# arpg/ba

Hardware: AMD Instinct MI355X
Metric: Gauss-Newton iterations/sec (higher is better)
Workload: dtype f64; 1 GPU; BASELINE.json configs[3]: 10000 poses / 1000000 landmarks / 10000000 reprojection residuals, pinhole, LmSize=1, PoseSize=6, Gauss-Newton (no dogleg), 2 anchor poses inactive; poses=10000, landmarks=1000000, residuals=10000000, reduced_system_n=59988, driver=phase calls of the C-ABI (include/ba_hip.h), parallelism=single GPU

## Files before the change

### ba_amd/csrc/engine.h

```cpp
#pragma once
#include <hip/hip_runtime.h>
#include <stdint.h>
#include <string>
#include <vector>

#include "../../include/ba_hip.h"
#include "structure.h"
#include "ordering.h"
#include "selinv.h"
#include "marg.h"
#include "pcg.h"
#include "dist_plan.h"

namespace bae {

template <typename T>
struct DBuf {
  T* p = nullptr;
  size_t n = 0;
  hipError_t alloc(size_t count) {
    if (count <= n && p) return hipSuccess;
    release();
    if (count == 0) { n = 0; return hipSuccess; }
    hipError_t err = hipMalloc((void**)&p, count * sizeof(T));
    if (err == hipSuccess) n = count;
    return err;
  }
  void release() {
    if (p) (void)hipFree(p);
    p = nullptr;
    n = 0;
  }
  size_t bytes() const { return n * sizeof(T); }
};
template <typename T>
// ... 69 lines not shown
  DBuf<double> obs_w0;
  DBuf<uint8_t> obs_cond;
  DBuf<uint2> wave_rng;
  DBuf<uint32_t> tile_ptr;
  DBuf<uint2> tile_ref;
  DBuf<uint32_t> tile_order;
  DBuf<uint4> tile_desc;
  uint32_t n_tile_order = 0;
  uint64_t tile_order_version = ~0ull;
  uint64_t tile_order_plan = ~0ull;
  int dbg_assemble_variant = 5;
  int dbg_host_structure = 0;
  int dbg_linearize_variant = 0;
  int dbg_tile_order = 0;
  int dbg_imu_wave = -1;
  int dbg_all_tiles = 0;
  DBuf<uint2> pair_ent;
  DBuf<uint32_t> pose_ptr, pose_mid;
  DBuf<uint32_t> pose_ent;
  DBuf<uint8_t> nzL;
  bool nzL_valid = false;
  std::vector<uint8_t> nzL_host;
  uint64_t nzL_version = 0;
  std::vector<uint8_t> nzS_host;
  DBuf<uint32_t> dist_srows;
  std::vector<uint32_t> dist_srows_off;
  uint64_t dist_srows_version = ~0ull;
  DBuf<uint32_t> dist_rows;
  std::vector<uint32_t> dist_rows_off;
  uint64_t dist_rows_version = ~0ull;
  DBuf<double> dist_msg;
  DistPlan dist_plan;
  uint64_t dist_plan_version = ~0ull;
  std::string dist_layout_name;
  DBuf<uint32_t> dist_tiles;
  uint64_t dist_sp_version = ~0ull;
  std::vector<uint32_t> dist_sp_send, dist_sp_recv;
  std::vector<size_t> dist_sp_send_off, dist_sp_recv_off;
  DBuf<uint4> dist_sp_srect, dist_sp_rrect;
  DBuf<uint2> dist_pairs;
  std::vector<uint32_t> dist_pair_first;
  uint32_t dist_npairs = 0;
  DBuf<uint32_t> dist_sq_list;
  DBuf<double> dist_usend, dist_urecv;
  DBuf<double> dist_ssend, dist_srecv;
  DBuf<double> dist_back;
// ... 203 lines not shown
int launch_calib_border(Engine* e);
int launch_calib_dogleg(Engine* e, int gn_available, ba_hip_dogleg_scalars* out);
int launch_begin_solve(Engine* e);
int launch_end_solve(Engine* e);
int launch_residual_vectors(Engine* e, double* d_r2);
int launch_residuals(Engine* e, int mode);
int launch_landmarks(Engine* e, double c_huber, int use_robust);
int launch_gather_S(Engine* e);
int launch_pack_lower(Engine* e, int unpack);
size_t packed_lower_count(uint32_t n_pad);
int launch_backsub(Engine* e);
int launch_compose_step(Engine* e, double coef_rhs, double coef_gn, double* norms2_host);
int launch_apply_step(Engine* e);
int launch_dogleg(Engine* e, int gn_available, double* h7, bool skip_jrhs);
int select_kth(Engine* e, const double* d_values, uint32_t n_local, uint64_t k, double* out);
int sum_partials(Engine* e, uint32_t nparts, uint32_t ncomp, double* host_out, bool cross_shard = true);
void defer_begin(Engine* e);
int defer_flush(Engine* e);
int launch_imu_early(Engine* e, double c_huber_proj);
int launch_posepose_build(Engine* e, double c_huber_proj, double* h3);
int launch_posepose_eval(Engine* e, double* h3);
int launch_posepose_jrhs(Engine* e, double* out);
int cholesky_solve(Engine* e, double* dA, uint32_t n, uint32_t ld, double* dx, int* status,
                   const uint8_t* nz_tiles);
int factor_tile_pattern(Engine* e);
uint32_t choose_kout(uint32_t nblk);
bool dist_solve_enabled(const Engine* e);
int dist_reduce_scatter_S(Engine* e);
int launch_imu_residual_vectors(Engine* e, double* d_r15);
int build_tile_order(Engine* e);
int build_tile_desc(Engine* e);
int dist_assembly_tiles(Engine* e, std::vector<uint8_t>* need);
int build_lists_device(Engine* e, const std::function<void(const char*)>& stage);
int order_poses(Engine* e, std::vector<uint64_t>* proj_edges, double device_ms);
bool ordering_wants_graph(const Engine* e);
int dist_broadcast(Engine* e, double* buf, size_t count, int root, hipStream_t s);
struct DistXfer { double* buf; size_t count; int peer; bool send; };
int dist_exchange(Engine* e, const std::vector<DistXfer>& x, bool side, hipStream_t s);
int dist_allreduce_stream(Engine* e, double* buf, size_t count, hipStream_t s);
void comm_release(Engine* e);
int check_solve_residual(Engine* e, const double* dS, const double* dx, const double* db, double* out2);
int cholesky_solve_dist(Engine* e, double* dA, uint32_t ld, double* dx, int* status, const uint8_t* nz);
int trailing_marginals(Engine* e, const double* dA, uint32_t ld, uint32_t first, uint32_t K, double* cov);
int marginals_compute(Engine* e);
int marginals_gather(Engine* e, uint32_t n, const std::vector<uint32_t>& ra, const std::vector<uint32_t>& rb, int Da,
                     int Db, double* out);
int marginals_landmarks(Engine* e, uint32_t n, const uint32_t* ids, double* out);
void marginals_release(Engine* e);
int leverages_run(Engine* e, uint32_t n, const uint32_t* ids, double* out);
// ... 14 lines not shown
```

### ba_amd/csrc/engine.hip

```cpp
#include "engine.h"
#include <chrono>
#include <functional>
#include <memory>
#include <thread>

#include <algorithm>
#include <cmath>
#include <cstdlib>
#include <cstring>
#include <numeric>

#include "dmath.h"
#include "dpose.h"

namespace bae {

int Engine::fail(hipError_t e, const char* what) {
  err = std::string(what) + ": " + hipGetErrorString(e);
  return -(int)(e == hipSuccess ? 1 : e);
}
void Engine::prof_collect() {
  auto drain = [](std::vector<std::pair<hipEvent_t, hipEvent_t>>& v, double& ms, uint32_t& n) {
    for (auto& p : v) {
      (void)hipEventSynchronize(p.second);
// ... 1020 lines not shown
      uint32_t a = 0;
      for (uint32_t p = 0; p < st.P; ++p)
        if (st.pose_opt[p] >= 0) {
          for (uint32_t d = 0; d < D; ++d) nat[(size_t)st.pose_opt[p] * D + d] = a * D + d;
          ++a;
        }
      for (uint32_t k = 0; k < st.K; ++k) nat[st.np + k] = st.Pact * D + k;
      build_pcg_coarse(e->pcg_plan, nat, st.Pact, D, st.K, e->pcg_opt.coarse_aggregate);
      e->pcg_coarse_built = e->pcg_opt.coarse_aggregate;
    }
    if ((rc = pcg_solve_device(e, e->A.p, st.n, st.ld, e->rhs_sc.p, e->pcg_plan, e->nzS_host, e->pcg_blk, e->pcg_blocks, rebuild,
                               e->pcg_opt, e->gn_p.p, &e->pcg_stats, &status))) return rc;
    e->factored = false;
    e->pcg_last = e->pcg_solved = true;
  } else if (st.n > 0 && !skip) {
    if (e->opt.keep_reduced_system) {
      BAE_HIP(e->A_keep.alloc((size_t)st.ld * st.ld));
      BAE_HIP(hipMemcpyAsync(e->A_keep.p, e->A.p, (size_t)st.ld * st.ld * sizeof(double),
                             hipMemcpyDeviceToDevice, e->stream));
    }
    if (!e->nzL_valid && (rc = factor_tile_pattern(e))) return rc;
    if (dist_solve_enabled(e)) {
      if ((rc = cholesky_solve_dist(e, e->A.p, st.ld, e->gn_p.p, &status, e->nzL.p))) return rc;
    } else if ((rc = cholesky_solve(e, e->A.p, st.n, st.ld, e->gn_p.p, &status, e->nzL.p))) return rc;
    e->factored = true;
    e->factor_foreign = false;
  }
  e->timers.solve = t.stop_ms();
  EventTimer tb(e);
  if ((rc = launch_backsub(e))) return rc;
  e->timers.back_substitution = tb.stop_ms();
  return status ? BA_HIP_FACTORIZATION_ERROR : 0;
}

int ba_hip_dogleg_terms(ba_hip_engine* h, int gn_available, ba_hip_dogleg_scalars* out) {
  ENG(h);
  NEED_FINAL();
  BAE_HIP(hipSetDevice(e->device));
  memset(out, 0, sizeof(*out));
  double* dh = e->dog_h;
  const bool reuse = gn_available && e->dog_jrhs_valid;
  defer_begin(e);
  int rc = launch_dogleg(e, gn_available, dh, reuse);
  if (!rc && !reuse) rc = launch_posepose_jrhs(e, dh + 7);
  if (!rc && !reuse) rc = launch_priors_jrhs(e, &e->prior_jrhs_h);
  const int rf = defer_flush(e);
  if (rc || rf) { e->dog_jrhs_valid = false; return rc ? rc : rf; }
// ... 669 lines not shown
  if (err != hipSuccess) rc = e->fail(err, "hipMemcpy");
  if (!rc && shard_allreduce(e, d.p, count, dtype) != 0) rc = e->fail_msg("allreduce hook failed");
  if (!rc && (err = hipMemcpy(host, d.p, count * 8, hipMemcpyDeviceToHost)) != hipSuccess) rc = e->fail(err, "hipMemcpy");
  d.release();
  return rc;
}

int ba_hip_get_comm_stats(ba_hip_engine* h, ba_hip_comm_stats* out) {
  ENG(h);
  if (!out) return e->fail_msg("null output");
  *out = e->cstats;
  return 0;
}

int ba_hip_reset_comm_stats(ba_hip_engine* h) {
  ENG(h);
  memset(&e->cstats, 0, sizeof(e->cstats));
  return 0;
}

int ba_hip_dist_plan_stats(uint32_t nblk, const uint8_t* nz_lower, int nranks, const char* layout, uint32_t kout,
                           ba_hip_dist_plan_stats_t* out) {
  if (!out || nranks < 1 || nblk == 0) return -1;
  const uint32_t G = kout ? kout : choose_kout(nblk);
  OwnMap map;
  std::string name;
  if (!build_own_map((uint32_t)nranks, layout, G, &map, &name)) return -1;
  const DistPlanStats s = dist_plan_stats(build_dist_plan(nblk, map, nz_lower));
  out->factor_bytes = s.factor_bytes;
  out->chain_recv_max = s.chain_recv_max; out->chain_recv_total = s.chain_recv_total;
  out->side_recv_max = s.side_recv_max; out->side_recv_total = s.side_recv_total;
  out->chain_sent_total = s.chain_sent_total; out->side_sent_total = s.side_sent_total;
  out->recv_max = s.recv_max; out->backward_allreduce_bytes = s.backward_allreduce_bytes;
  out->messages_chain = s.messages_chain; out->messages_side = s.messages_side;
  out->panels = s.panels; out->ranks = s.ranks; out->classes = s.classes; out->kout = G;
  return 0;
}

int ba_hip_get_factor_tile_pattern(ba_hip_engine* h, uint32_t nblk, uint8_t* nz_lower) {
  ENG(h);
  NEED_FINAL();
  if (!e->nzL_valid) {
    BAE_HIP(hipSetDevice(e->device));
    const int rc = factor_tile_pattern(e);
    if (rc) return rc;
  }
  if (e->nzL_host.size() != (size_t)nblk * nblk) return e->fail_msg("tile count mismatch");
  memcpy(nz_lower, e->nzL_host.data(), e->nzL_host.size());
  return 0;
}

int ba_hip_solve_is_distributed(ba_hip_engine* h) {
  if (!h) return 0;
  return dist_solve_enabled(reinterpret_cast<Engine*>(h)) ? 1 : 0;
}

int ba_hip_set_pose_ordering(ba_hip_engine* h, int mode) {
  ENG(h);
  if (mode != kOrderNatural && mode != kOrderAuto && mode != kOrderUser)
    return e->fail_msg("ba_hip_set_pose_ordering: unknown mode");
  if (mode != kOrderNatural && e->ordering_refused())
    return e->fail_msg("pose ordering is not available on a sharded engine (all-reduce hook, collectives hook or communicator set)");
  e->order_mode = mode;
  return 0;
}

int ba_hip_set_reduced_solver(ba_hip_engine* h, int mode, const ba_hip_pcg_options* o) {
  ENG(h);
  if (mode != BA_HIP_SOLVER_DIRECT && mode != BA_HIP_SOLVER_PCG) return e->fail_msg("ba_hip_set_reduced_solver: unknown mode");
  if (mode == BA_HIP_SOLVER_PCG) {
    if (e->pcg_refused())
      return e->fail_msg("the PCG solver is not available on a sharded engine (all-reduce hook, collectives hook or communicator set)");
    ba_hip_pcg_options v = {};
    v.rel_tolerance = 1e-6;
    if (o) v = *o;
    if (!(v.rel_tolerance > 0.0) || !(v.rel_tolerance < 1.0))
      return e->fail_msg("ba_hip_set_reduced_solver: rel_tolerance must lie in (0, 1)");
// ... 297 lines not shown
        if (!t && tile_map && r / 64 != c / 64) {
          e->err = "ba_hip_tile_solve: entry (" + std::to_string(r) + ", " + std::to_string(c) + ") is nonzero but tile (" +
                   std::to_string(r / 64) + ", " + std::to_string(c / 64) + ") is not in the tile map";
          return -1;
        }
        t = 1;
      }
    }
  for (uint32_t i = 0; i < nt; ++i) nz[(size_t)i * nt + i] = 1;
  for (uint32_t r = n; r < ld; ++r) A[(size_t)r * ld + r] = 1.0;
  for (uint32_t c = 0; c < n; ++c) A[(size_t)ld * ld + c] = b[c];
  tile_symbolic_factor(nz, nt);
  if (nz_factor) std::copy(nz.begin(), nz.end(), nz_factor);
  DBuf<double> dA, dx;
  DBuf<uint8_t> dnz;
  BAE_HIP(dA.alloc(A.size()));
  BAE_HIP(dx.alloc(ld));
  BAE_HIP(dnz.alloc(nz.size()));
  BAE_HIP(e->flags.alloc(16));
  BAE_HIP(hipMemcpy(dA.p, A.data(), A.size() * 8, hipMemcpyHostToDevice));
  BAE_HIP(hipMemcpy(dnz.p, nz.data(), nz.size(), hipMemcpyHostToDevice));
  int status = 0;
  e->factor_foreign = true;
  int rc = cholesky_solve(e, dA.p, n, ld, dx.p, &status, dnz.p);
  if (rc == 0) {
    std::vector<double> xx(ld);
    hipError_t err = hipDeviceSynchronize();
    if (err == hipSuccess) err = hipMemcpy(xx.data(), dx.p, (size_t)ld * 8, hipMemcpyDeviceToHost);
    if (err == hipSuccess && factor) err = hipMemcpy(factor, dA.p, (size_t)ld * ld * 8, hipMemcpyDeviceToHost);
    if (err == hipSuccess && dsgn) err = hipMemcpy(dsgn, e->invdiag.p, (size_t)ld * 8, hipMemcpyDeviceToHost);
    if (err == hipSuccess && linvT)
      err = hipMemcpy(linvT, e->invdiag.p + ld, (size_t)nt * 64 * 64 * 8, hipMemcpyDeviceToHost);
    if (err != hipSuccess) rc = e->fail(err, "hipMemcpy");
    for (uint32_t i = 0; i < n; ++i) x[i] = xx[i];
  }
  dA.release(); dx.release(); dnz.release();
  if (rc) return rc;
  return status ? BA_HIP_FACTORIZATION_ERROR : 0;
}

int ba_hip_select_kth(ba_hip_engine* h, uint32_t n, const double* values, uint32_t k, double* out) {
  ENG(h);
  BAE_HIP(hipSetDevice(e->device));
  DBuf<double> dv;
  BAE_HIP(dv.alloc(std::max<uint32_t>(n, 1)));
  BAE_HIP(e->hist.alloc(2048 + 8));
  if (n) BAE_HIP(hipMemcpy(dv.p, values, (size_t)n * 8, hipMemcpyHostToDevice));
// ... 7 lines not shown
```

### ba_amd/csrc/hostcheck.cpp

```cpp
#include <vector>
#include "dmath.h"
using namespace bad;

static Rt rt_from7(const double* p) {
  Rt t;
  t.R = quat_to_rot(p[3], p[4], p[5], p[6]);
  t.t = v3(p[0], p[1], p[2]);
  return t;
}

static double g_hostcheck_fov_w = 0.0;
extern "C" void ba_hostcheck_set_fov(double w) { g_hostcheck_fov_w = w; }
static Cam cam_from4(const double* cam4) {
  Cam c = {cam4[0], cam4[1], cam4[2], cam4[3], g_hostcheck_fov_w, g_hostcheck_fov_w != 0.0 ? 1 : 0};
  return c;
}

static int g_hostcheck_variant = 1;
extern "C" void ba_hostcheck_set_variant(int v) { g_hostcheck_variant = v; }

extern "C" void ba_hostcheck_proj_jacobians(int lm_dim, const double* cam4, const double* z,
                                            const double* x, const double* t_wp_m7,
                                            const double* t_vs_m7, const double* t_wp_r7,
                                            const double* t_vs_r7, int same_pose, double* r2,
// ... 575 lines not shown
        for (int x = 0; x < 6; ++x)
          rows[(WO + k) * 6 + x] = (rows[x] * Jl[k] + rows[6 + x] * Jl[LM + k]) * sw;
      if (LM == 1) {
        double* lr = &frow[((size_t)st.lrow_base + 2 * l) * 6];
        for (int x = 0; x < 6; ++x) lr[x] += (rows[12 + x] * Jl[0] + rows[18 + x] * Jl[1]) * sw;
      }
      if (K > 0)
        for (int x = 0; x < K; ++x)
          crow[(2 * (size_t)O + l) * 6 + x] += (crow[2 * (size_t)s * 6 + x] * Jl[0] + crow[(2 * (size_t)s + 1) * 6 + x] * Jl[1]) * sw;
    }
  }
  LeverHostIn in;
  in.LM = LM; in.D = D; in.K = K; in.L = L; in.O = O; in.np = st.np; in.n = st.n; in.lrow_base = st.lrow_base;
  in.lm_ptr = st.lm_ptr.data(); in.obs_pose = st.obs_pose.data(); in.lm_ref_pose = lm_ref_pose;
  in.pose_opt = st.pose_opt.data(); in.lm_opt = st.lm_opt.data();
  in.frow = frow.data(); in.obs_jl = obs_jl.data(); in.crow = K > 0 ? crow.data() : nullptr;
  in.sigma = sigma;
  std::vector<double> sorted((size_t)O * 4, 0.0);
  leverage_host(in, variant, sorted.data());
  for (uint32_t s = 0; s < O; ++s)
    for (int i = 0; i < 4; ++i) out[4 * (size_t)st.obs_perm[s] + i] = sorted[4 * (size_t)s + i];
  return 0;
}
```

### ba_amd/csrc/k_chol.hip

```cpp
#include "engine.h"
#include <cstdlib>
#include <algorithm>
#include <vector>

namespace bae {

static const int NB = 64;
static const int LDT = NB + 2;

typedef double double4_t __attribute__((ext_vector_type(4)));

__device__ __forceinline__ double readlane_f64(double v, int lane) {
  int lo = __double2loint(v), hi = __double2hiint(v);
  lo = __builtin_amdgcn_readlane(lo, lane);
  hi = __builtin_amdgcn_readlane(hi, lane);
  return __hiloint2double(hi, lo);
}

static const int LDM = 18;

static const int KC2 = 16;
#ifndef BAE_LDK2
#define BAE_LDK2 (KC2 + 2)
#endif
// ... 252 lines not shown
    while ((uint64_t)(sr + 1) * (sr + 2) / 2 <= t) ++sr;
    while ((uint64_t)sr * (sr + 1) / 2 > t) --sr;
    const uint32_t sc = t - (uint32_t)((uint64_t)sr * (sr + 1) / 2);
    const uint32_t R = (sr << sbl) + (within >> sbl), C = (sc << sbl) + (within & ((1u << sbl) - 1u));
    if (C > R) return;
    c = c0 + C;
    i = c0 + R;
    if (i > nblk || c >= nblk) return;
  } else {
    c = c0 + blockIdx.y;
    i = c + blockIdx.x;
    if (i > nblk) return;
  }
  if (!own_tile(own, i, c, nblk)) return;
  update_tile(A, ld, nblk, i, c, kb0, kb1, dsgn, colneg, nz, X, Y, klist);
}

static const int NB2 = 128;
#ifdef BAE_TIME128
__device__ unsigned long long* g_t128_buf = nullptr;
__device__ unsigned int g_t128_n = 0;
static const unsigned int T128_CAP = 1u << 21, T128_REC = 6;
#endif
template <bool RECT, bool LIST = false>
__global__ void __launch_bounds__(256, 2)
k_update128(double* __restrict__ A, uint32_t ld, uint32_t nblk, uint32_t c0, uint32_t m2, uint32_t kb0,
            uint32_t kb1, const double* __restrict__ dsgn, const int* __restrict__ colneg, uint32_t sbl,
            const uint8_t* __restrict__ nz, const OwnMap own,
            uint32_t nrow64, uint32_t r0, uint32_t rect_cols) {
  __shared__ double X[2][NB2][LDK2];
  __shared__ double Y[2][NB2][LDK2];
  __shared__ uint32_t klist[32];
  if (blockIdx.x < nrow64) {
    const uint32_t mcols = RECT ? 2 * rect_cols : nblk - c0, y = blockIdx.x / mcols;
    const uint32_t c = c0 + blockIdx.x % mcols, i = nblk - y;
    if (y > ((nblk - r0) & 1u) || c > i || c >= nblk) return;
    if (!own_tile(own, i, c, nblk)) return;
    update_tile(A, ld, nblk, i, c, kb0, kb1, dsgn, colneg, nz, reinterpret_cast<double(*)[NB][LDK2]>(&X[0][0][0]),
                reinterpret_cast<double(*)[NB][LDK2]>(&Y[0][0][0]), klist);
    return;
  }
  const uint32_t b = blockIdx.x - nrow64;
  uint32_t R, C;
  if constexpr (LIST) {
    const uint32_t gb = own.G >> 1, per = gb * gb;
    const uint32_t pr = b / per, within = b - pr * per;
    const uint2* pairs = reinterpret_cast<const uint2*>(((unsigned long long)own.pairs_hi << 32) | own.pairs_lo);
    const uint2 bp = pairs[pr];
    const uint32_t base = c0 / own.G;
    R = (bp.x - base) * gb + within / gb;
    C = (bp.y - base) * gb + within % gb;
    if (C > R || R >= m2) return;
  } else if (RECT) {
    R = b / rect_cols;
    C = b % rect_cols;
    if (R >= m2) return;
  } else {
    const uint32_t xcd = b & 7u, slot = b >> 3;
    const uint32_t t = (slot >> (2 * sbl)) * 8u + xcd, within = slot & ((1u << (2 * sbl)) - 1u);
    uint32_t sr_ = (uint32_t)((sqrt(8.0 * (double)t + 1.0) - 1.0) * 0.5);
    while ((uint64_t)(sr_ + 1) * (sr_ + 2) / 2 <= t) ++sr_;
    while ((uint64_t)sr_ * (sr_ + 1) / 2 > t) --sr_;
    const uint32_t sc_ = t - (uint32_t)((uint64_t)sr_ * (sr_ + 1) / 2);
    R = (sr_ << sbl) + (within >> sbl);
    C = (sc_ << sbl) + (within & ((1u << sbl) - 1u));
    if (C > R || R >= m2) return;
  }
// ... 964 lines not shown
  if (nz.size() != (size_t)nt * nt) nz.assign((size_t)nt * nt, 1);
  static const bool dense = getenv("BA_HIP_DENSE") != nullptr;
  if (dense) std::fill(nz.begin(), nz.end(), 1);
  if (e->sharded() && !dense) {
    std::vector<double> cnt(nz.begin(), nz.end());
    DBuf<double> d;
    BAE_HIP(d.alloc(cnt.size()));
    BAE_HIP(hipMemcpy(d.p, cnt.data(), cnt.size() * sizeof(double), hipMemcpyHostToDevice));
    if (shard_allreduce(e, d.p, cnt.size(), 0) != 0) { d.release(); return e->fail_msg("allreduce hook failed"); }
    BAE_HIP(hipMemcpy(cnt.data(), d.p, cnt.size() * sizeof(double), hipMemcpyDeviceToHost));
    d.release();
    for (size_t i = 0; i < nz.size(); ++i) nz[i] = cnt[i] > 0.5 ? 1 : 0;
  }
  e->nzS_host = nz;
  tile_symbolic_factor(nz, nt);
  BAE_HIP(e->nzL.alloc(nz.size()));
  BAE_HIP(hipMemcpy(e->nzL.p, nz.data(), nz.size(), hipMemcpyHostToDevice));
  e->nzL_host = nz;
  e->nzL_version++;
  e->nzL_valid = true;
  return 0;
}

uint32_t choose_kout(uint32_t nblk) {
  const char* ke = getenv("BA_HIP_KOUT");
  const uint32_t kout_env = ke ? (uint32_t)atoi(ke) : 0;
  return kout_env ? kout_env : (nblk >= 400 ? 16u : nblk >= 256 ? 8u : 4u);
}

bool dist_solve_enabled(const Engine* e) {
  static const bool off = getenv("BA_HIP_NO_DIST_SOLVE") != nullptr;
  return e->coll && e->sharded() && !e->opt.keep_reduced_system && !off;
}

__global__ void __launch_bounds__(256)
k_copy_panel_rows(double* __restrict__ A, uint32_t ld, const uint32_t* __restrict__ tiles, uint32_t ntiles,
                  uint32_t n_pad, uint32_t c0, uint32_t w, double* __restrict__ buf, int unpack) {
  const uint32_t r = blockIdx.x;
  const uint32_t arow = (r < ntiles * NB) ? tiles[r >> 6] * NB + (r & 63u) : n_pad;
  double* row = A + (size_t)arow * ld + c0;
  double* brow = buf + (size_t)r * w;
  for (uint32_t cc = threadIdx.x; cc < w; cc += 256) {
    if (unpack) row[cc] = brow[cc];
    else brow[cc] = row[cc];
  }
}

static const uint32_t KIN = 4;
static void launch_panel_chain(hipStream_t s, double* dA, uint32_t ld, uint32_t nblk, uint32_t J, uint32_t Jend,
                               double* dsgn, double* opbuf, int* colneg, int* flags, const uint8_t* nz,
// ... 54 lines not shown
                                     uint32_t ncols, uint32_t kb0, uint32_t kb1, double* dsgn, double* opbuf,
                                     int* colneg, int* flags, const uint8_t* nz, bool factor = true) {
  static const bool no128 = getenv("BA_HIP_NO128") != nullptr;
  const uint32_t r0 = c0 + ncols;
  auto step_update = factor ? k_step_update<true> : k_step_update<false>;
  static const uint32_t min_rows =
      getenv("BA_HIP_BULK_FULL_M") ? (uint32_t)std::max(16, atoi(getenv("BA_HIP_BULK_FULL_M"))) : 128u;
  if (!no128 && r0 + min_rows <= nblk && ncols % 2u == 0 && c0 % 2u == 0) {
    const uint32_t m = nblk - r0, m2 = m / 2, rect_cols = ncols / 2;
    hipLaunchKernelGGL(step_update, dim3(ncols, ncols), dim3(256), 0, s, dA, ld, nblk, c0, kb0, kb1, dsgn, opbuf,
                       colneg, flags, nz, r0, (const uint32_t*)nullptr);
    const uint32_t nrow64 = (ncols * (1 + (m & 1u)) + 7) / 8 * 8;
    hipLaunchKernelGGL(k_update128<true>, dim3(nrow64 + m2 * rect_cols), dim3(256), 0, s, dA, ld, nblk, c0, m2, kb0, kb1,
                       (const double*)dsgn, (const int*)colneg, 0u, nz, own_map_single(), nrow64, r0, rect_cols);
    return;
  }
  hipLaunchKernelGGL(step_update, dim3(nblk - c0 + 1, ncols), dim3(256), 0, s, dA, ld, nblk, c0, kb0, kb1, dsgn,
                     opbuf, colneg, flags, nz, nblk + 1u, (const uint32_t*)nullptr);
}

static void launch_bulk_update(Engine* e, hipStream_t s, double* dA, uint32_t ld, uint32_t nblk, uint32_t a_end,
                                   uint32_t J, uint32_t Jend, const double* dsgn, const int* colneg,
                                   const uint8_t* nz, bool full, const OwnMap& own, const uint2* pairs = nullptr,
                                   uint32_t npairs = 0) {
  static const bool no128 = getenv("BA_HIP_NO128") != nullptr;
  static const uint32_t sbl = getenv("BA_HIP_SBL") ? (uint32_t)atoi(getenv("BA_HIP_SBL")) : 3u;
  const uint32_t m = nblk - a_end;
  if (full && !no128 && m >= 16 && (a_end % 2u) == 0 && (own.n <= 1 || own.G % 2u == 0)) {
    const uint32_t m2 = m / 2, sbl2 = 2, sbe2 = 1u << sbl2;
    const uint32_t nsr = (m2 + sbe2 - 1) / sbe2, nsb = nsr * (nsr + 1) / 2;
    const uint32_t nrow64 = (m * (1 + (m & 1u)) + 7) / 8 * 8;
    if (e) e->prof_begin(e->ev_syrk, s);
    if (pairs && own.n > 1 && a_end % own.G == 0) {
      OwnMap ol = own;
      ol.pairs_lo = (uint32_t)(reinterpret_cast<unsigned long long>(pairs) & 0xffffffffull);
      ol.pairs_hi = (uint32_t)(reinterpret_cast<unsigned long long>(pairs) >> 32);
      const uint32_t per = (own.G / 2) * (own.G / 2);
      hipLaunchKernelGGL((k_update128<false, true>), dim3(nrow64 + npairs * per), dim3(256), 0, s, dA, ld, nblk,
                         a_end, m2, J, Jend, dsgn, colneg, sbl2, nz, ol, nrow64, a_end, 0u);
    } else {
      hipLaunchKernelGGL(k_update128<false>, dim3(nrow64 + ((nsb + 7) / 8) * 8 * sbe2 * sbe2), dim3(256), 0, s, dA, ld, nblk,
                         a_end, m2, J, Jend, dsgn, colneg, sbl2, nz, own, nrow64, a_end, 0u);
    }
    if (e) e->prof_end(e->ev_syrk, s);
    return;
  }
  const uint32_t sbe = 1u << sbl;
  const uint32_t nsr = (m + 1 + sbe - 1) / sbe, nsb = nsr * (nsr + 1) / 2;
  const uint32_t grid1 = ((nsb + 7) / 8) * 8 * sbe * sbe;
  const int swzf = 1 | (int)(sbl << 8);
  if (e) e->prof_begin(e->ev_syrk, s);
  if (full)
    hipLaunchKernelGGL(k_update2<false>, dim3(grid1), dim3(256), 0, s, dA, ld, nblk, a_end, J, Jend, dsgn, colneg,
                       swzf, nz, own);
  else
    hipLaunchKernelGGL(k_update2<true>, dim3(grid1), dim3(256), 0, s, dA, ld, nblk, a_end, J, Jend, dsgn, colneg,
                       swzf, nz, own);
  if (e) e->prof_end(e->ev_syrk, s);
}

static int ensure_dist_plan(Engine* e, uint32_t nblk, bool pat) {
  const uint32_t KOUT = choose_kout(nblk);
  const char* lay_env = getenv("BA_HIP_DIST_LAYOUT");
  const uint64_t want = (pat ? e->nzL_version : 0) * 1024 + KOUT * 4 + (pat ? 1 : 0);
  if (e->dist_plan_version == want && e->dist_plan.nblk == nblk && e->dist_plan.map.n == (uint32_t)e->nranks &&
      e->dist_plan.map.rank == (uint32_t)e->rank)
    return 0;
  OwnMap map;
  std::string why;
  if (!build_own_map((uint32_t)e->nranks, lay_env, KOUT, &map, &e->dist_layout_name, &why)) {
    e->err = "distributed solve: " + why;
    return -1;
  }
  map.rank = (uint32_t)e->rank;
  e->dist_plan = build_dist_plan(nblk, map, pat ? e->nzL_host.data() : nullptr, e->nranks == 1);
  BAE_HIP(e->dist_tiles.alloc(std::max<size_t>(e->dist_plan.tiles.size(), 1)));
  if (!e->dist_plan.tiles.empty())
    BAE_HIP(hipMemcpy(e->dist_tiles.p, e->dist_plan.tiles.data(), e->dist_plan.tiles.size() * sizeof(uint32_t),
                      hipMemcpyHostToDevice));
  {
    const DistPlan& pl = e->dist_plan;
    std::vector<uint2> pairs;
    e->dist_pair_first.assign(pl.nb + 1, 0);
    for (uint32_t bc = 0; bc < pl.nb; ++bc) {
      if (bc >= 2) e->dist_pair_first[bc - 2] = (uint32_t)pairs.size();
// ... 535 lines not shown
    for (uint32_t r = 0; r < b; ++r)
      for (uint32_t c = 0; c <= r; ++c) G[(size_t)(a + r) * K + a + c] = tile[(size_t)c * NB + r];
    std::vector<double> Lba((size_t)b * a);
    BAE_HIP(hipMemcpy2D(Lba.data(), a * sizeof(double), dA + (size_t)(t + 1) * NB * ld + (size_t)t * NB + o,
                        ld * sizeof(double), a * sizeof(double), b, hipMemcpyDeviceToHost));
    for (uint32_t r = 0; r < b; ++r)
      for (uint32_t c = 0; c < a; ++c) {
        double s = 0.0;
        for (uint32_t x = 0; x < b; ++x)
          for (uint32_t y = 0; y < a; ++y) s += G[(size_t)(a + r) * K + a + x] * Lba[(size_t)x * a + y] * G[(size_t)y * K + c];
        G[(size_t)(a + r) * K + c] = -s;
      }
  }
  for (uint32_t r = 0; r < K; ++r)
    for (uint32_t c = 0; c < K; ++c) {
      double s = 0.0;
      for (uint32_t j = 0; j < K; ++j) s += G[(size_t)j * K + r] * sg[j] * G[(size_t)j * K + c];
      cov[(size_t)r * K + c] = s;
    }
  return 0;
}

int cholesky_solve(Engine* e, double* dA, uint32_t n, uint32_t ld, double* dx, int* status,
                   const uint8_t* nz) {
  (void)n;
  const uint32_t nblk = ld / NB;
  BAE_HIP(e->invdiag.alloc((size_t)nblk * NB + (size_t)nblk * NB * NB + (size_t)nblk * NOPV * 64 +
                           (nblk + 1) / 2));
  double* dsgn = e->invdiag.p;
  double* linvT = dsgn + (size_t)nblk * NB;
  double* opbuf = linvT + (size_t)nblk * NB * NB;
  int* colneg = reinterpret_cast<int*>(opbuf + (size_t)nblk * NOPV * 64);
  static const bool no_lookahead = getenv("BA_HIP_NO_LOOKAHEAD") != nullptr;
  static const bool bulk_full = getenv("BA_HIP_BULK_FULL") != nullptr;
  static const uint32_t bulk_full_m =
      getenv("BA_HIP_BULK_FULL_M") ? (uint32_t)atoi(getenv("BA_HIP_BULK_FULL_M")) : 128u;
  hipStream_t s0 = e->stream, s1 = no_lookahead ? e->stream : e->stream2;
  const uint32_t KOUT = choose_kout(nblk);
  const uint32_t npanels = (nblk + KOUT - 1) / KOUT;
  while (e->ev_panel.size() < npanels) {
    hipEvent_t a, b;
    BAE_HIP(hipEventCreateWithFlags(&a, hipEventDisableTiming));
    BAE_HIP(hipEventCreateWithFlags(&b, hipEventDisableTiming));
    e->ev_panel.push_back(a);
    e->ev_bulk.push_back(b);
  }
  { const int src = setup_status_block(e, dA, ld, s0); if (src) return src; }
#ifdef BAE_TIME128
  static unsigned long long* t128_dev = nullptr;
  if (getenv("BA_HIP_TRACE_FILE")) {
    if (!t128_dev) {
      BAE_HIP(hipMalloc(&t128_dev, (size_t)T128_CAP * T128_REC * sizeof(unsigned long long)));
      BAE_HIP(hipMemcpyToSymbol(HIP_SYMBOL(g_t128_buf), &t128_dev, sizeof(t128_dev)));
    }
    const unsigned int zero = 0;
    BAE_HIP(hipMemcpyToSymbol(HIP_SYMBOL(g_t128_n), &zero, sizeof(zero)));
  }
#endif
  const char* sqe = getenv("BA_HIP_SQUARE");
  const bool sq = nblk < 512 && sqe && atoi(sqe) != 0;
  if (sq) {
    if (!e->square_attr_set) {
      BAE_HIP(hipFuncSetAttribute(reinterpret_cast<const void*>(k_square), hipFuncAttributeMaxDynamicSharedMemorySize,
                                  (int)sizeof(SquareLds)));
      BAE_HIP(hipFuncSetAttribute(reinterpret_cast<const void*>(k_rowpanel), hipFuncAttributeMaxDynamicSharedMemorySize,
                                  (int)sizeof(RowPanelLds)));
      e->square_attr_set = true;
    }
  } else {
    hipLaunchKernelGGL(k_step_update<true>, dim3(1, 1), dim3(256), 0, s0, dA, ld, nblk, 0u, 0u, 0u, dsgn, opbuf,
                       colneg, e->flags.p, nz, nblk + 1u, (const uint32_t*)nullptr);
  }
  int prev_bulk = -1;
  uint32_t pj = 0;
  for (uint32_t J = 0; J < nblk; J += KOUT, ++pj) {
    const uint32_t Jend = J + KOUT < nblk ? J + KOUT : nblk;
    launch_panel_chain(s0, dA, ld, nblk, J, Jend, dsgn, opbuf, colneg, e->flags.p, nz, nullptr, 0, false, sq);
    if (Jend >= nblk) break;
    BAE_HIP(hipEventRecord(e->ev_panel[pj], s0));
    const uint32_t a_end = Jend + KOUT < nblk ? Jend + KOUT : nblk;
    if (prev_bulk >= 0) BAE_HIP(hipStreamWaitEvent(s0, e->ev_bulk[prev_bulk], 0));
    launch_next_panel_update(s0, dA, ld, nblk, Jend, a_end - Jend, J, Jend, dsgn, opbuf, colneg, e->flags.p, nz, !sq);
    if (a_end < nblk) {
      BAE_HIP(hipStreamWaitEvent(s1, e->ev_panel[pj], 0));
      const uint32_t m = nblk - a_end;
      launch_bulk_update(e, s1, dA, ld, nblk, a_end, J, Jend, dsgn, colneg, nz,
                         no_lookahead || bulk_full || m >= bulk_full_m, own_map_single());
      BAE_HIP(hipEventRecord(e->ev_bulk[pj], s1));
      prev_bulk = (int)pj;
      if (e->profiling) {
        double tiles = 0.0;
        for (uint32_t kb = J; kb < Jend; ++kb) {
          double mk = (double)(nblk - a_end);
          if (nz && e->nzL_host.size() == (size_t)nblk * nblk) {
            mk = 0.0;
            for (uint32_t r = a_end; r < nblk; ++r) mk += e->nzL_host[(size_t)r * nblk + kb];
          }
          tiles += mk * (mk + 1) / 2 + mk;
        }
        e->kstats.syrk_flops += tiles * 2.0 * NB * NB * NB;
      }
    }
  }
  BAE_HIP(hipGetLastError());
  hipLaunchKernelGGL(k_linvT, dim3(nblk), dim3(256), 0, s0, (const double*)opbuf, (const double*)dsgn,
                       linvT);
  launch_backward(s0, dA, ld, nblk, (const double*)linvT, dx, nz);
  BAE_HIP(hipGetLastError());
  int st = 0;
  BAE_HIP(hipMemcpyAsync(&st, e->flags.p, sizeof(int), hipMemcpyDeviceToHost, s0));
// ... 21 lines not shown
```

### ba_amd/hipapi.py

```python
import ctypes as C
import os
import subprocess

import numpy as np

_HERE = os.path.dirname(os.path.abspath(__file__))
LIB_PATH = os.path.join(_HERE, "lib", "libba_hip.so")
if os.environ.get("BA_AMD_LIB"):
    LIB_PATH = os.path.abspath(os.environ["BA_AMD_LIB"])

dp = C.POINTER(C.c_double)
u32p = C.POINTER(C.c_uint32)
u8p = C.POINTER(C.c_uint8)
u16p = C.POINTER(C.c_uint16)


class Options(C.Structure):
    _fields_ = [("projection_outlier_threshold", C.c_double),
                ("use_robust_norm_for_proj_residuals", C.c_int32),
                ("use_robust_norm_for_inertial_residuals", C.c_int32),
                ("use_triangular_matrices", C.c_int32), ("keep_reduced_system", C.c_int32),
                ("gyro_sigma", C.c_double), ("accel_sigma", C.c_double),
                ("gyro_bias_sigma", C.c_double), ("accel_bias_sigma", C.c_double),
                ("pivot_rel_tolerance", C.c_double)]
# ... 126 lines not shown
    "ba_hip_set_projection_residuals", "ba_hip_set_unary_residuals",
    "ba_hip_set_binary_residuals", "ba_hip_set_imu_residuals", "ba_hip_set_inertial_covariance_once", "ba_hip_set_imu_noise", "ba_hip_integrate_imu", "ba_hip_set_gravity",
    "ba_hip_finalize", "ba_hip_begin_solve", "ba_hip_set_pose_masks", "ba_hip_linearize",
    "ba_hip_solve_gn", "ba_hip_dogleg_terms", "ba_hip_compose_step", "ba_hip_apply_step",
    "ba_hip_rollback", "ba_hip_eval_residuals", "ba_hip_end_solve", "ba_hip_get_poses",
    "ba_hip_get_landmarks", "ba_hip_get_landmark_flags", "ba_hip_num_pose_params",
    "ba_hip_num_lm_params", "ba_hip_get_S", "ba_hip_get_rhs", "ba_hip_get_delta_gn",
    "ba_hip_get_step", "ba_hip_get_proj_weights", "ba_hip_get_proj_residuals", "ba_hip_get_imu_residuals", "ba_hip_get_imu_errors", "ba_hip_get_timers", "ba_hip_get_unary_scales", "ba_hip_device_buffer",
    "ba_hip_set_allreduce", "ba_hip_set_collectives", "ba_hip_solve_is_distributed", "ba_hip_dense_solve", "ba_hip_select_kth", "ba_hip_set_profiling",
    "ba_hip_get_kernel_stats", "ba_hip_check_solve", "ba_hip_get_structure_stats", "ba_hip_debug_set", "ba_hip_set_conditioning_residuals",
    "ba_hip_get_conditioning_error", "ba_hip_comm_unique_id", "ba_hip_comm_init", "ba_hip_comm_destroy", "ba_hip_allreduce_host", "ba_hip_get_proj_jacobians",
    "ba_hip_set_calibration", "ba_hip_num_calib_params", "ba_hip_get_cameras", "ba_hip_get_calib_jacobians", "ba_hip_get_calibration_marginals", "ba_hip_set_landmark_ref_pixels", "ba_hip_get_camera_params",
    "ba_hip_set_camera_models", "ba_hip_get_camera_fov",
    "ba_hip_integrate_imu_jacobians", "ba_hip_imu_pose_derivative", "ba_hip_imu_integrate_pose", "ba_hip_lie",
    "ba_hip_get_comm_stats", "ba_hip_reset_comm_stats", "ba_hip_dist_plan_stats", "ba_hip_get_factor_tile_pattern",
    "ba_hip_set_pose_ordering", "ba_hip_set_pose_permutation", "ba_hip_get_pose_ordering", "ba_hip_get_pose_group_graph",
    "ba_hip_compute_marginals", "ba_hip_get_pose_marginals", "ba_hip_get_pose_pair_marginals",
    "ba_hip_get_calibration_block_marginals", "ba_hip_get_landmark_marginals", "ba_hip_get_marginal_stats",
    "ba_hip_release_marginals", "ba_hip_get_joint_marginals", "ba_hip_get_joint_marginal_stats",
    "ba_hip_set_dense_priors", "ba_hip_get_prior_errors", "ba_hip_marginalize", "ba_hip_get_marginalization",
    "ba_hip_release_marginalization", "ba_hip_set_unary_scales",
    "ba_hip_set_reduced_solver", "ba_hip_get_pcg_stats", "ba_hip_pcg_solve", "ba_hip_tile_solve",
    "ba_hip_get_pcg_coarse_stats", "ba_hip_get_pcg_coarse",
    "ba_hip_get_projection_leverages", "ba_hip_get_leverage_stats",
]

ORDER_NATURAL, ORDER_AUTO, ORDER_USER = 0, 1, 2
SOLVER_DIRECT, SOLVER_PCG = 0, 1


def build(force=False):
    src = os.path.join(_HERE, "csrc")
    if force:
        subprocess.check_call(["make", "-C", src, "clean", "-s"])
    subprocess.check_call(["make", "-C", src, "-j4", "-s"])
    return LIB_PATH


_lib = None


def lib():
    global _lib
    if _lib is None:
        if not os.path.exists(LIB_PATH):
            raise RuntimeError(
                "ba_amd: %s is missing — build the HIP extension first "
# ... 414 lines not shown
        self._chk(self.L.ba_hip_set_allreduce(self.h, self._cb, None, int(rank), int(nranks)))

    def set_collectives(self, fn):
        if fn is None:
            self._cb2 = None
            self._chk(self.L.ba_hip_set_collectives(self.h, None, None))
            return
        self._cb2 = COLLECTIVE_FN(lambda ctx, op, ptr, count, root: int(fn(op, ptr, count, root)))
        self._chk(self.L.ba_hip_set_collectives(self.h, self._cb2, None))

    @staticmethod
    def comm_unique_id():
        buf = C.create_string_buffer(128)
        if lib().ba_hip_comm_unique_id(buf) != 0:
            raise HipError("ba_hip_comm_unique_id failed (librccl not loadable?)")
        return buf.raw

    def comm_init(self, unique_id, rank, nranks):
        self._chk(self.L.ba_hip_comm_init(self.h, C.c_char_p(unique_id), int(rank), int(nranks)))

    def comm_destroy(self):
        self._chk(self.L.ba_hip_comm_destroy(self.h))

    def solve_is_distributed(self):
        return bool(self.L.ba_hip_solve_is_distributed(self.h))

    def comm_stats(self, reset=False):
        out = CommStats()
        self._chk(self.L.ba_hip_get_comm_stats(self.h, C.byref(out)))
        if reset:
            self._chk(self.L.ba_hip_reset_comm_stats(self.h))
        return {k: getattr(out, k) for k, _ in CommStats._fields_}

    def factor_tile_pattern(self):
        nblk = (self.num_pose_params() + self.num_calib_params() + 63) // 64
        nblk = max(nblk, 1)
        out = np.zeros((nblk, nblk), dtype=np.uint8)
        self._chk(self.L.ba_hip_get_factor_tile_pattern(self.h, nblk, out.ctypes.data_as(C.POINTER(C.c_uint8))))
        return out

    def set_reduced_solver(self, mode, rel_tolerance=1e-6, max_iterations=0, check_every=0, coarse_aggregate=0):
        if int(mode) == SOLVER_DIRECT:
            self._chk(self.L.ba_hip_set_reduced_solver(self.h, SOLVER_DIRECT, None))
            return
        o = PcgOptions(float(rel_tolerance), int(max_iterations), int(check_every), int(coarse_aggregate))
        self._chk(self.L.ba_hip_set_reduced_solver(self.h, int(mode), C.byref(o)))
# ... 57 lines not shown
```

### include/ba_hip.h

```cpp
#ifndef BA_HIP_H
#define BA_HIP_H
#include <stddef.h>
#include <stdint.h>
#ifdef __cplusplus
extern "C" {
#endif

#define BA_HIP_OK 0
#define BA_HIP_FACTORIZATION_ERROR 4
#define BA_HIP_SOLVER_ERROR 5

typedef struct ba_hip_engine ba_hip_engine;

typedef struct {
  double projection_outlier_threshold;
  int32_t use_robust_norm_for_proj_residuals;
  int32_t use_robust_norm_for_inertial_residuals;
  int32_t use_triangular_matrices;
  int32_t keep_reduced_system;
  double gyro_sigma, accel_sigma, gyro_bias_sigma, accel_bias_sigma;
  double pivot_rel_tolerance;
} ba_hip_options;

typedef struct {
// ... 137 lines not shown
int ba_hip_comm_destroy(ba_hip_engine* e);
typedef struct {
  double chain_bytes_sent, chain_bytes_recv;
  double side_bytes_sent, side_bytes_recv;
  double reduce_scatter_bytes;
  double allreduce_bytes;
  uint64_t chain_messages, side_messages, factorisations;
} ba_hip_comm_stats;
int ba_hip_get_comm_stats(ba_hip_engine* e, ba_hip_comm_stats* out);
int ba_hip_reset_comm_stats(ba_hip_engine* e);
typedef struct {
  double factor_bytes;
  double chain_recv_max, chain_recv_total;
  double side_recv_max, side_recv_total;
  double chain_sent_total, side_sent_total;
  double recv_max;
  double backward_allreduce_bytes;
  uint32_t messages_chain, messages_side, panels, ranks, classes, kout;
} ba_hip_dist_plan_stats_t;
int ba_hip_dist_plan_stats(uint32_t nblk, const uint8_t* nz_lower, int nranks, const char* layout, uint32_t kout,
                           ba_hip_dist_plan_stats_t* out);
int ba_hip_get_factor_tile_pattern(ba_hip_engine* e, uint32_t nblk, uint8_t* nz_lower);
int ba_hip_solve_is_distributed(ba_hip_engine* e);

#define BA_HIP_ORDER_NATURAL 0
#define BA_HIP_ORDER_AUTO 1
#define BA_HIP_ORDER_USER 2
typedef struct {
  int32_t mode;
  int32_t candidate;
  uint32_t group_size;
  uint32_t num_groups;
  uint64_t tile_products_natural;
  uint64_t tile_products_chosen;
  double host_ms;
  double device_ms;
} ba_hip_ordering_stats;
int ba_hip_set_pose_ordering(ba_hip_engine* e, int mode);
int ba_hip_set_pose_permutation(ba_hip_engine* e, const uint32_t* opt_of_natural, uint32_t n);
int ba_hip_get_pose_ordering(ba_hip_engine* e, uint32_t* opt_of_natural, ba_hip_ordering_stats* st);
int ba_hip_get_pose_group_graph(ba_hip_engine* e, uint32_t* ptr, uint32_t* adj, uint32_t* num_groups,
                                uint32_t* num_edges);

typedef struct {
  double selinv_ms;
  double landmark_ms;
// ... 98 lines not shown
```

Before: 1.724 iterations/sec.

## Launch Cholesky bulk updates over precomputed live-block lists and retune panel width

Precomputes on the host, per panel, a compact list of trailing 128x128 block pairs whose update is nonzero given the factor tile sparsity pattern. The list is cached by pattern version and uploaded, and the bulk SYRK kernel then launches only those blocks instead of the full lower-triangular grid. Separately, the default panel width (kout) for the single-GPU path grows for large block counts (nblk around 938 here gives 20), while the distributed path keeps the old choice. This saves many empty workgroups in sparse trailing updates, at the cost of host-side list construction whenever the pattern changes and of different panel/lookahead behaviour.

```diff
diff --git a/ba_amd/csrc/bulk_list.h b/ba_amd/csrc/bulk_list.h
--- /dev/null
+++ b/ba_amd/csrc/bulk_list.h
@@ -0,0 +1,106 @@
+#pragma once
+#include <stdint.h>
+#include <algorithm>
+#include <vector>
+
+namespace bae {
+
+static const uint32_t kBulkSentinel = 0xffffffffu;
+static const uint32_t kBulkSbl = 2;
+
+inline uint32_t bulk_entry(uint32_t R, uint32_t C) { return R | (C << 16); }
+
+struct BulkLaunch {
+  uint32_t J = 0, Jend = 0, a_end = 0, m2 = 0;
+  bool listed = false;
+  size_t off = 0;
+  uint32_t len = 0;
+  uint32_t live = 0;
+  uint32_t full_grid = 0;
+};
+
+struct BulkLists {
+  std::vector<BulkLaunch> launches;
+  std::vector<uint32_t> ent;
+  uint64_t live = 0, full_grid = 0, listed = 0;
+};
+
+inline bool bulk_block_live(const uint8_t* nz, uint32_t nblk, uint32_t a_end, uint32_t J, uint32_t Jend, uint32_t R,
+                            uint32_t C) {
+  const size_t i = a_end + 2 * (size_t)R, c = a_end + 2 * (size_t)C;
+  for (uint32_t k = J; k < Jend; ++k)
+    if ((nz[i * nblk + k] | nz[(i + 1) * nblk + k]) && (nz[c * nblk + k] | nz[(c + 1) * nblk + k])) return true;
+  return false;
+}
+
+inline void build_bulk_lists(const uint8_t* nz, uint32_t nblk, uint32_t kout, uint32_t thr, BulkLists& out) {
+  out = BulkLists();
+  thr = std::max(thr, 16u);
+  const uint32_t sbe = 1u << kBulkSbl;
+  std::vector<uint32_t> lane[8];
+  for (uint32_t J = 0; J < nblk; J += kout) {
+    const uint32_t Jend = std::min(J + kout, nblk);
+    if (Jend >= nblk) break;
+    const uint32_t a_end = std::min(Jend + kout, nblk);
+    BulkLaunch L;
+    L.J = J; L.Jend = Jend; L.a_end = a_end; L.off = out.ent.size();
+    const uint32_t m = nblk - a_end;
+    if (a_end < nblk && m >= thr && (a_end % 2u) == 0 && m / 2 <= 0xffffu) {
+      L.listed = true;
+      const uint32_t m2 = m / 2, nsr = (m2 + sbe - 1) / sbe, nsb = nsr * (nsr + 1) / 2;
+      L.m2 = m2;
+      L.full_grid = ((nsb + 7) / 8) * 8 * sbe * sbe;
+      for (auto& l : lane) l.clear();
+      uint32_t q = 0;
+      for (uint32_t sr = 0; sr < nsr; ++sr)
+        for (uint32_t sc = 0; sc <= sr; ++sc) {
+          std::vector<uint32_t>& l = lane[q & 7u];
+          const size_t before = l.size();
+          for (uint32_t within = 0; within < sbe * sbe; ++within) {
+            const uint32_t R = sr * sbe + (within >> kBulkSbl), C = sc * sbe + (within & (sbe - 1));
+            if (C > R || R >= m2) continue;
+            if (bulk_block_live(nz, nblk, a_end, J, Jend, R, C)) l.push_back(bulk_entry(R, C));
+          }
+          if (l.size() != before) ++q;
+        }
+      size_t longest = 0;
+      for (auto& l : lane) { longest = std::max(longest, l.size()); L.live += (uint32_t)l.size(); }
+      L.len = (uint32_t)(8 * longest);
+      out.ent.resize(L.off + L.len, kBulkSentinel);
+      for (uint32_t x = 0; x < 8; ++x)
+        for (size_t s = 0; s < lane[x].size(); ++s) out.ent[L.off + 8 * s + x] = lane[x][s];
+      out.live += L.live; out.full_grid += L.full_grid; out.listed += L.len;
+    }
+    out.launches.push_back(L);
+  }
+}
+
+inline bool bulk_lists_valid(const BulkLists& b, uint32_t nblk) {
+  for (const BulkLaunch& L : b.launches) {
+    if (!L.listed) continue;
+    if (L.len % 8u || L.off + L.len > b.ent.size() || L.a_end + 2 * (size_t)L.m2 > nblk) return false;
+    for (uint32_t x = 0; x < L.len; ++x) {
+      const uint32_t v = b.ent[L.off + x];
+      if (v == kBulkSentinel) continue;
+      const uint32_t R = v & 0xffffu, C = v >> 16;
+      if (R >= L.m2 || C > R) return false;
+    }
+  }
+  return true;
+}
+
+struct BulkListCache {
+  uint64_t version = 0;
+  uint32_t nblk = 0, kout = 0, thr = 0;
+  BulkLists lists;
+  uint64_t builds = 0;
+  bool ensure(const uint8_t* nz, uint64_t ver, uint32_t nblk_, uint32_t kout_, uint32_t thr_) {
+    if (ver && ver == version && nblk_ == nblk && kout_ == kout && thr_ == thr) return false;
+    build_bulk_lists(nz, nblk_, kout_, thr_, lists);
+    version = ver; nblk = nblk_; kout = kout_; thr = thr_;
+    ++builds;
+    return true;
+  }
+};
+
+}
diff --git a/ba_amd/csrc/engine.h b/ba_amd/csrc/engine.h
--- a/ba_amd/csrc/engine.h
+++ b/ba_amd/csrc/engine.h
@@ -11,6 +11,7 @@
 #include "marg.h"
 #include "pcg.h"
 #include "dist_plan.h"
+#include "bulk_list.h"
 
 namespace bae {
 
@@ -126,6 +127,8 @@
   bool nzL_valid = false;
   std::vector<uint8_t> nzL_host;
   uint64_t nzL_version = 0;
+  BulkListCache bulk_lists;
+  DBuf<uint32_t> bulk_lists_dev;
   std::vector<uint8_t> nzS_host;
   DBuf<uint32_t> dist_srows;
   std::vector<uint32_t> dist_srows_off;
@@ -375,9 +378,10 @@
 int launch_posepose_eval(Engine* e, double* h3);
 int launch_posepose_jrhs(Engine* e, double* out);
 int cholesky_solve(Engine* e, double* dA, uint32_t n, uint32_t ld, double* dx, int* status,
-                   const uint8_t* nz_tiles);
+                   const uint8_t* nz_tiles, const uint8_t* nz_tiles_host = nullptr, uint64_t nz_version = 0);
 int factor_tile_pattern(Engine* e);
 uint32_t choose_kout(uint32_t nblk);
+uint32_t choose_kout_dist(uint32_t nblk);
 bool dist_solve_enabled(const Engine* e);
 int dist_reduce_scatter_S(Engine* e);
 int launch_imu_residual_vectors(Engine* e, double* d_r15);
diff --git a/ba_amd/csrc/engine.hip b/ba_amd/csrc/engine.hip
--- a/ba_amd/csrc/engine.hip
+++ b/ba_amd/csrc/engine.hip
@@ -1066,7 +1066,8 @@
     if (!e->nzL_valid && (rc = factor_tile_pattern(e))) return rc;
     if (dist_solve_enabled(e)) {
       if ((rc = cholesky_solve_dist(e, e->A.p, st.ld, e->gn_p.p, &status, e->nzL.p))) return rc;
-    } else if ((rc = cholesky_solve(e, e->A.p, st.n, st.ld, e->gn_p.p, &status, e->nzL.p))) return rc;
+    } else if ((rc = cholesky_solve(e, e->A.p, st.n, st.ld, e->gn_p.p, &status, e->nzL.p, e->nzL_host.data(),
+                                    e->nzL_version))) return rc;
     e->factored = true;
     e->factor_foreign = false;
   }
@@ -1782,7 +1783,7 @@
 int ba_hip_dist_plan_stats(uint32_t nblk, const uint8_t* nz_lower, int nranks, const char* layout, uint32_t kout,
                            ba_hip_dist_plan_stats_t* out) {
   if (!out || nranks < 1 || nblk == 0) return -1;
-  const uint32_t G = kout ? kout : choose_kout(nblk);
+  const uint32_t G = kout ? kout : choose_kout_dist(nblk);
   OwnMap map;
   std::string name;
   if (!build_own_map((uint32_t)nranks, layout, G, &map, &name)) return -1;
@@ -1813,6 +1814,16 @@
 int ba_hip_solve_is_distributed(ba_hip_engine* h) {
   if (!h) return 0;
   return dist_solve_enabled(reinterpret_cast<Engine*>(h)) ? 1 : 0;
+}
+
+int ba_hip_bulk_list_stats(ba_hip_engine* h, uint64_t out[5]) {
+  ENG(h);
+  if (!out) return e->fail_msg("null output");
+  const BulkLists& b = e->bulk_lists.lists;
+  uint64_t listed = 0;
+  for (const BulkLaunch& L : b.launches) listed += L.listed ? 1 : 0;
+  out[0] = e->bulk_lists.builds; out[1] = listed; out[2] = b.listed; out[3] = b.live; out[4] = b.full_grid;
+  return 0;
 }
 
 int ba_hip_set_pose_ordering(ba_hip_engine* h, int mode) {
@@ -2156,7 +2167,7 @@
   BAE_HIP(hipMemcpy(dnz.p, nz.data(), nz.size(), hipMemcpyHostToDevice));
   int status = 0;
   e->factor_foreign = true;
-  int rc = cholesky_solve(e, dA.p, n, ld, dx.p, &status, dnz.p);
+  int rc = cholesky_solve(e, dA.p, n, ld, dx.p, &status, dnz.p, nz.data(), 0);
   if (rc == 0) {
     std::vector<double> xx(ld);
     hipError_t err = hipDeviceSynchronize();
diff --git a/ba_amd/csrc/hostcheck.cpp b/ba_amd/csrc/hostcheck.cpp
--- a/ba_amd/csrc/hostcheck.cpp
+++ b/ba_amd/csrc/hostcheck.cpp
@@ -621,3 +621,24 @@
     for (int i = 0; i < 4; ++i) out[4 * (size_t)st.obs_perm[s] + i] = sorted[4 * (size_t)s + i];
   return 0;
 }
+
+#include "bulk_list.h"
+
+extern "C" int ba_hostcheck_bulk_lists(uint32_t nblk, const uint8_t* nz, uint64_t version, uint32_t kout, uint32_t thr,
+                                       uint32_t* launches, uint32_t max_launches, uint32_t* entries,
+                                       uint64_t max_entries, uint64_t* counts) {
+  static bae::BulkListCache cache;
+  if (!nblk || !nz || !kout || kout > 64) return -1;
+  cache.ensure(nz, version, nblk, kout, thr);
+  const bae::BulkLists& b = cache.lists;
+  counts[0] = cache.builds; counts[1] = b.launches.size(); counts[2] = b.ent.size(); counts[3] = b.live;
+  if (!bae::bulk_lists_valid(b, nblk)) return -2;
+  if (b.launches.size() > max_launches || b.ent.size() > max_entries) return -1;
+  for (size_t l = 0; l < b.launches.size(); ++l) {
+    const bae::BulkLaunch& L = b.launches[l];
+    const uint32_t row[8] = {L.J, L.Jend, L.a_end, L.m2, L.listed ? 1u : 0u, (uint32_t)L.off, L.len, L.full_grid};
+    std::copy(row, row + 8, launches + 8 * l);
+  }
+  std::copy(b.ent.begin(), b.ent.end(), entries);
+  return (int)b.launches.size();
+}
diff --git a/ba_amd/csrc/k_chol.hip b/ba_amd/csrc/k_chol.hip
--- a/ba_amd/csrc/k_chol.hip
+++ b/ba_amd/csrc/k_chol.hip
@@ -298,7 +298,7 @@
 __device__ unsigned int g_t128_n = 0;
 static const unsigned int T128_CAP = 1u << 21, T128_REC = 6;
 #endif
-template <bool RECT, bool LIST = false>
+template <bool RECT, bool LIST = false, bool LIVE = false>
 __global__ void __launch_bounds__(256, 2)
 k_update128(double* __restrict__ A, uint32_t ld, uint32_t nblk, uint32_t c0, uint32_t m2, uint32_t kb0,
             uint32_t kb1, const double* __restrict__ dsgn, const int* __restrict__ colneg, uint32_t sbl,
@@ -318,7 +318,13 @@
   }
   const uint32_t b = blockIdx.x - nrow64;
   uint32_t R, C;
-  if constexpr (LIST) {
+  if constexpr (LIVE) {
+    const uint32_t* blocks = reinterpret_cast<const uint32_t*>(((unsigned long long)own.pairs_hi << 32) | own.pairs_lo);
+    const uint32_t ent = blocks[b];
+    if (ent == 0xffffffffu) return;
+    R = ent & 0xffffu;
+    C = ent >> 16;
+  } else if constexpr (LIST) {
     const uint32_t gb = own.G >> 1, per = gb * gb;
     const uint32_t pr = b / per, within = b - pr * per;
     const uint2* pairs = reinterpret_cast<const uint2*>(((unsigned long long)own.pairs_hi << 32) | own.pairs_lo);
@@ -1329,10 +1335,20 @@
   return 0;
 }
 
+uint32_t choose_kout_dist(uint32_t nblk) {
+  const char* ke = getenv("BA_HIP_KOUT");
+  const uint32_t kout_env = ke ? (uint32_t)atoi(ke) : 0;
+  return kout_env ? kout_env : (nblk >= 400 ? 16u : nblk >= 256 ? 8u : 4u);
+}
+
 uint32_t choose_kout(uint32_t nblk) {
   const char* ke = getenv("BA_HIP_KOUT");
   const uint32_t kout_env = ke ? (uint32_t)atoi(ke) : 0;
-  return kout_env ? kout_env : (nblk >= 400 ? 16u : nblk >= 256 ? 8u : 4u);
+  if (kout_env) return kout_env;
+  static const struct { uint32_t from, kout; } table[] = {{1758, 32}, {1055, 24}, {704, 20}, {400, 16}, {256, 8}, {0, 4}};
+  for (const auto& t : table)
+    if (nblk >= t.from) return t.kout;
+  return 4u;
 }
 
 bool dist_solve_enabled(const Engine* e) {
@@ -1433,12 +1449,12 @@
 static void launch_bulk_update(Engine* e, hipStream_t s, double* dA, uint32_t ld, uint32_t nblk, uint32_t a_end,
                                    uint32_t J, uint32_t Jend, const double* dsgn, const int* colneg,
                                    const uint8_t* nz, bool full, const OwnMap& own, const uint2* pairs = nullptr,
-                                   uint32_t npairs = 0) {
+                                   uint32_t npairs = 0, const uint32_t* live = nullptr, uint32_t nlive = 0) {
   static const bool no128 = getenv("BA_HIP_NO128") != nullptr;
   static const uint32_t sbl = getenv("BA_HIP_SBL") ? (uint32_t)atoi(getenv("BA_HIP_SBL")) : 3u;
   const uint32_t m = nblk - a_end;
   if (full && !no128 && m >= 16 && (a_end % 2u) == 0 && (own.n <= 1 || own.G % 2u == 0)) {
-    const uint32_t m2 = m / 2, sbl2 = 2, sbe2 = 1u << sbl2;
+    const uint32_t m2 = m / 2, sbl2 = kBulkSbl, sbe2 = 1u << sbl2;
     const uint32_t nsr = (m2 + sbe2 - 1) / sbe2, nsb = nsr * (nsr + 1) / 2;
     const uint32_t nrow64 = (m * (1 + (m & 1u)) + 7) / 8 * 8;
     if (e) e->prof_begin(e->ev_syrk, s);
@@ -1448,6 +1464,12 @@
       ol.pairs_hi = (uint32_t)(reinterpret_cast<unsigned long long>(pairs) >> 32);
       const uint32_t per = (own.G / 2) * (own.G / 2);
       hipLaunchKernelGGL((k_update128<false, true>), dim3(nrow64 + npairs * per), dim3(256), 0, s, dA, ld, nblk,
+                         a_end, m2, J, Jend, dsgn, colneg, sbl2, nz, ol, nrow64, a_end, 0u);
+    } else if (live && nz && own.n <= 1) {
+      OwnMap ol = own;
+      ol.pairs_lo = (uint32_t)(reinterpret_cast<unsigned long long>(live) & 0xffffffffull);
+      ol.pairs_hi = (uint32_t)(reinterpret_cast<unsigned long long>(live) >> 32);
+      hipLaunchKernelGGL((k_update128<false, false, true>), dim3(nrow64 + nlive), dim3(256), 0, s, dA, ld, nblk,
                          a_end, m2, J, Jend, dsgn, colneg, sbl2, nz, ol, nrow64, a_end, 0u);
     } else {
       hipLaunchKernelGGL(k_update128<false>, dim3(nrow64 + ((nsb + 7) / 8) * 8 * sbe2 * sbe2), dim3(256), 0, s, dA, ld, nblk,
@@ -1471,7 +1493,7 @@
 }
 
 static int ensure_dist_plan(Engine* e, uint32_t nblk, bool pat) {
-  const uint32_t KOUT = choose_kout(nblk);
+  const uint32_t KOUT = choose_kout_dist(nblk);
   const char* lay_env = getenv("BA_HIP_DIST_LAYOUT");
   const uint64_t want = (pat ? e->nzL_version : 0) * 1024 + KOUT * 4 + (pat ? 1 : 0);
   if (e->dist_plan_version == want && e->dist_plan.nblk == nblk && e->dist_plan.map.n == (uint32_t)e->nranks &&
@@ -2053,7 +2075,7 @@
 }
 
 int cholesky_solve(Engine* e, double* dA, uint32_t n, uint32_t ld, double* dx, int* status,
-                   const uint8_t* nz) {
+                   const uint8_t* nz, const uint8_t* nz_host, uint64_t nz_version) {
   (void)n;
   const uint32_t nblk = ld / NB;
   BAE_HIP(e->invdiag.alloc((size_t)nblk * NB + (size_t)nblk * NB * NB + (size_t)nblk * NOPV * 64 +
@@ -2077,6 +2099,20 @@
     e->ev_bulk.push_back(b);
   }
   { const int src = setup_status_block(e, dA, ld, s0); if (src) return src; }
+  const char* ble = getenv("BA_HIP_BULK_LIST");
+  const bool use_lists = nz && nz_host && KOUT <= 64 && !(ble && atoi(ble) == 0);
+  if (use_lists) {
+    const uint32_t thr = (no_lookahead || bulk_full) ? 16u : std::max(bulk_full_m, 16u);
+    if (e->bulk_lists.ensure(nz_host, nz_version, nblk, KOUT, thr)) {
+      e->bulk_lists.version = 0;
+      if (!bulk_lists_valid(e->bulk_lists.lists, nblk)) return e->fail_msg("bulk block list: entry outside the trailing matrix");
+      const std::vector<uint32_t>& ent = e->bulk_lists.lists.ent;
+      BAE_HIP(e->bulk_lists_dev.alloc(std::max<size_t>(ent.size(), 1)));
+      if (!ent.empty())
+        BAE_HIP(hipMemcpy(e->bulk_lists_dev.p, ent.data(), ent.size() * sizeof(uint32_t), hipMemcpyHostToDevice));
+      e->bulk_lists.version = nz_version;
+    }
+  }
 #ifdef BAE_TIME128
   static unsigned long long* t128_dev = nullptr;
   if (getenv("BA_HIP_TRACE_FILE")) {
@@ -2115,8 +2151,11 @@
     if (a_end < nblk) {
       BAE_HIP(hipStreamWaitEvent(s1, e->ev_panel[pj], 0));
       const uint32_t m = nblk - a_end;
+      const BulkLaunch* bl = use_lists && pj < e->bulk_lists.lists.launches.size() ? &e->bulk_lists.lists.launches[pj] : nullptr;
+      const bool listed = bl && bl->listed && bl->J == J && bl->a_end == a_end;
       launch_bulk_update(e, s1, dA, ld, nblk, a_end, J, Jend, dsgn, colneg, nz,
-                         no_lookahead || bulk_full || m >= bulk_full_m, own_map_single());
+                         no_lookahead || bulk_full || m >= bulk_full_m, own_map_single(), nullptr, 0,
+                         listed ? e->bulk_lists_dev.p + bl->off : nullptr, listed ? bl->len : 0u);
       BAE_HIP(hipEventRecord(e->ev_bulk[pj], s1));
       prev_bulk = (int)pj;
       if (e->profiling) {
diff --git a/ba_amd/hipapi.py b/ba_amd/hipapi.py
--- a/ba_amd/hipapi.py
+++ b/ba_amd/hipapi.py
@@ -172,7 +172,7 @@
     "ba_hip_release_marginalization", "ba_hip_set_unary_scales",
     "ba_hip_set_reduced_solver", "ba_hip_get_pcg_stats", "ba_hip_pcg_solve", "ba_hip_tile_solve",
     "ba_hip_get_pcg_coarse_stats", "ba_hip_get_pcg_coarse",
-    "ba_hip_get_projection_leverages", "ba_hip_get_leverage_stats",
+    "ba_hip_get_projection_leverages", "ba_hip_get_leverage_stats", "ba_hip_bulk_list_stats",
 ]
 
 ORDER_NATURAL, ORDER_AUTO, ORDER_USER = 0, 1, 2
@@ -633,6 +633,11 @@
     def comm_destroy(self):
         self._chk(self.L.ba_hip_comm_destroy(self.h))
 
+    def bulk_list_stats(self):
+        out = (C.c_uint64 * 5)()
+        self._chk(self.L.ba_hip_bulk_list_stats(self.h, out))
+        return tuple(int(v) for v in out)
+
     def solve_is_distributed(self):
         return bool(self.L.ba_hip_solve_is_distributed(self.h))
 
diff --git a/include/ba_hip.h b/include/ba_hip.h
--- a/include/ba_hip.h
+++ b/include/ba_hip.h
@@ -183,6 +183,7 @@
                            ba_hip_dist_plan_stats_t* out);
 int ba_hip_get_factor_tile_pattern(ba_hip_engine* e, uint32_t nblk, uint8_t* nz_lower);
 int ba_hip_solve_is_distributed(ba_hip_engine* e);
+int ba_hip_bulk_list_stats(ba_hip_engine* e, uint64_t out[5]);
 
 #define BA_HIP_ORDER_NATURAL 0
 #define BA_HIP_ORDER_AUTO 1
```

Measured after the change: 1.734 iterations/sec, median of 6. No clear change (+0.6%).
